# KristinnVikarJ/nbody-simulation

Measured on AMD Instinct MI355X. Metric: pair-interactions/sec + ms/step at N=1M direct O(N^2) (force + integration step), higher is better.
Workload: dtype f32; 1 GPU; direct O(N^2) f32, N=1048576 bodies, seeded 2-D Plummer sphere, masses 1, dt=0.1, clamp=0.001 (BASELINE.json configs[2]); n_bodies=1048576, targets_per_gpu=1048576, n_ranks=1, entry=one process per GPU (sharding.py over nbody_direct_{prep,run}_dev), exchange=none, arith=AUTO (FAST kernel; EXACT on hazardous positions)

## Files before the change

nbody-simulation_amd/csrc/direct_mutual.hip:

```cpp
#include <hip/hip_runtime.h>
#include <stdint.h>

#include "direct_kernels.h"
#include "mutual_schedule.h"

namespace nbody {

namespace {

typedef float v2f __attribute__((ext_vector_type(2)));

constexpr int kWaves = 8;

constexpr int kSlice = kMutualSlice;
constexpr int kSliceCouples = kSlice / 2;
constexpr int kChunks = kSliceCouples / 64;
constexpr float kMarker = 1e30f;

__device__ __forceinline__ bool gate_open(const DirectArgs& a) { return a.run_state < 0 || a.flags[kFlagState] == a.run_state; }

__device__ __forceinline__ float4 couple_or_marker(const float4* c, int64_t k, int64_t n_couples) {
  return k < n_couples ? c[k] : make_float4(kMarker, kMarker, kMarker, kMarker);
}

#define NB_PX(K, H, D) "v_pk_add_f32 v[" D "], v[184:185], %[tx" #K "] op_sel:[0," #H "] op_sel_hi:[1," #H "] neg_lo:[0,1] neg_hi:[0,1]\n\t"
#define NB_PY(K, H, D) "v_pk_add_f32 v[" D "], v[186:187], %[ty" #K "] op_sel:[0," #H "] op_sel_hi:[1," #H "] neg_lo:[0,1] neg_hi:[0,1]\n\t"
#define NB_SQ(DX, DY, Q) "v_pk_mul_f32 v[" Q "], v[" DX "], v[" DX "]\n\tv_pk_fma_f32 v[" Q "], v[" DY "], v[" DY "], v[" Q "]\n\t"
#define NB_AD(XL, XH, YL, YH, SL, SH) "v_add_f32_e64 v" SL ", |v" XL "|, |v" YL "|\n\tv_add_f32_e64 v" SH ", |v" XH "|, |v" YH "|\n\t"
#define NB_DN(S, Q) "v_pk_fma_f32 v[" S "], v[" S "], v[" Q "], %[b]\n\t"
#define NB_RC(SL, SH) "v_rcp_f32_e32 v" SL ", v" SL "\n\tv_rcp_f32_e32 v" SH ", v" SH "\n\t"
#define NB_AC(T, DX, DY, S)                                                                                                          \
  "v_pk_fma_f32 %[ax" #T "], v[" DX "], v[" S "], %[ax" #T "]\n\t"                                                                    \
  "v_pk_fma_f32 v[188:189], v[" DX "], v[" S "], v[188:189] neg_lo:[1,0,0] neg_hi:[1,0,0]\n\t"                                                  \
  "v_pk_fma_f32 %[ay" #T "], v[" DY "], v[" S "], %[ay" #T "]\n\t"                                                                    \
  "v_pk_fma_f32 v[190:191], v[" DY "], v[" S "], v[190:191] neg_lo:[1,0,0] neg_hi:[1,0,0]\n\t"
#define NB_HALF(K0, K1, K2, K3, T0, T1, T2, T3, T4, T5, T6, T7)                                                                    \
  NB_PX(K0, 0, "192:193") NB_PX(K0, 1, "200:201") NB_PX(K1, 0, "208:209") NB_PX(K1, 1, "216:217")                                   \
  NB_PX(K2, 0, "224:225") NB_PX(K2, 1, "232:233") NB_PX(K3, 0, "240:241") NB_PX(K3, 1, "248:249")                                   \
  NB_PY(K0, 0, "194:195") NB_PY(K0, 1, "202:203") NB_PY(K1, 0, "210:211") NB_PY(K1, 1, "218:219")                                   \
  NB_PY(K2, 0, "226:227") NB_PY(K2, 1, "234:235") NB_PY(K3, 0, "242:243") NB_PY(K3, 1, "250:251")                                   \
  NB_SQ("192:193", "194:195", "196:197") NB_SQ("200:201", "202:203", "204:205") NB_SQ("208:209", "210:211", "212:213")             \
  NB_SQ("216:217", "218:219", "220:221") NB_SQ("224:225", "226:227", "228:229") NB_SQ("232:233", "234:235", "236:237")             \
  NB_SQ("240:241", "242:243", "244:245") NB_SQ("248:249", "250:251", "252:253")                                                    \
  "s_setprio 0\n\t"                                                                                                                \
  NB_AD("192", "193", "194", "195", "198", "199") NB_AD("200", "201", "202", "203", "206", "207")                                  \
  NB_AD("208", "209", "210", "211", "214", "215") NB_AD("216", "217", "218", "219", "222", "223")                                  \
  NB_AD("224", "225", "226", "227", "230", "231") NB_AD("232", "233", "234", "235", "238", "239")                                  \
  NB_AD("240", "241", "242", "243", "246", "247") NB_AD("248", "249", "250", "251", "254", "255")                                  \
  "s_setprio 1\n\t"                                                                                                                \
  NB_DN("198:199", "196:197") NB_DN("206:207", "204:205") NB_DN("214:215", "212:213") NB_DN("222:223", "220:221")                 \
  NB_DN("230:231", "228:229") NB_DN("238:239", "236:237") NB_DN("246:247", "244:245") NB_DN("254:255", "252:253")                 \
  NB_RC("198", "199")                                                                                                              \
  NB_RC("206", "207") NB_AC(T0, "192:193", "194:195", "198:199")                                                                   \
  NB_RC("214", "215") NB_AC(T1, "200:201", "202:203", "206:207")                                                                   \
  NB_RC("222", "223") NB_AC(T2, "208:209", "210:211", "214:215")                                                                   \
  NB_RC("230", "231") NB_AC(T3, "216:217", "218:219", "222:223")                                                                   \
  NB_RC("238", "239") NB_AC(T4, "224:225", "226:227", "230:231")                                                                   \
  NB_RC("246", "247") NB_AC(T5, "232:233", "234:235", "238:239")                                                                   \
  NB_RC("254", "255") NB_AC(T6, "240:241", "242:243", "246:247")                                                                   \
  NB_AC(T7, "248:249", "250:251", "254:255")
#define NB_ROT(R) "v_mov_b32_dpp " R ", " R " wave_ror:1 row_mask:0xf bank_mask:0xf\n\t"

__device__ __forceinline__ void mutual_steps(const v2f* tx, const v2f* ty, v2f* ax, v2f* ay, float4& rc, float4& sacc, int steps,
                                             unsigned long long bias2) {
  asm volatile("v_mov_b32 v184, %[r0]\n\tv_mov_b32 v185, %[r1]\n\tv_mov_b32 v186, %[r2]\n\tv_mov_b32 v187, %[r3]\n\t"
               "v_mov_b32 v188, %[o0]\n\tv_mov_b32 v189, %[o1]\n\tv_mov_b32 v190, %[o2]\n\tv_mov_b32 v191, %[o3]\n\t"
               "s_mov_b32 s88, %[n]\n"
               ".Lnb_mutual_%=:\n\t"
               NB_HALF(0, 1, 2, 3, 0, 1, 2, 3, 4, 5, 6, 7) NB_HALF(4, 5, 6, 7, 8, 9, 10, 11, 12, 13, 14, 15)
               NB_ROT("v184") NB_ROT("v185") NB_ROT("v186") NB_ROT("v187") NB_ROT("v188") NB_ROT("v189") NB_ROT("v190") NB_ROT("v191")
               "s_sub_u32 s88, s88, 1\n\t"
               "s_cmp_lg_u32 s88, 0\n\t"
               "s_cbranch_scc1 .Lnb_mutual_%=\n\t"
               "v_mov_b32 %[o0], v188\n\tv_mov_b32 %[o1], v189\n\tv_mov_b32 %[o2], v190\n\tv_mov_b32 %[o3], v191\n\t"
               "v_mov_b32 %[r0], v184\n\tv_mov_b32 %[r1], v185\n\tv_mov_b32 %[r2], v186\n\tv_mov_b32 %[r3], v187\n\t"
               : [ax0] "+v"(ax[0]), [ax1] "+v"(ax[1]), [ax2] "+v"(ax[2]), [ax3] "+v"(ax[3]), [ax4] "+v"(ax[4]), [ax5] "+v"(ax[5]),
                 [ax6] "+v"(ax[6]), [ax7] "+v"(ax[7]), [ax8] "+v"(ax[8]), [ax9] "+v"(ax[9]), [ax10] "+v"(ax[10]), [ax11] "+v"(ax[11]),
                 [ax12] "+v"(ax[12]), [ax13] "+v"(ax[13]), [ax14] "+v"(ax[14]), [ax15] "+v"(ax[15]),
                 [ay0] "+v"(ay[0]), [ay1] "+v"(ay[1]), [ay2] "+v"(ay[2]), [ay3] "+v"(ay[3]), [ay4] "+v"(ay[4]), [ay5] "+v"(ay[5]),
                 [ay6] "+v"(ay[6]), [ay7] "+v"(ay[7]), [ay8] "+v"(ay[8]), [ay9] "+v"(ay[9]), [ay10] "+v"(ay[10]), [ay11] "+v"(ay[11]),
                 [ay12] "+v"(ay[12]), [ay13] "+v"(ay[13]), [ay14] "+v"(ay[14]), [ay15] "+v"(ay[15]),
                 [o0] "+v"(sacc.x), [o1] "+v"(sacc.y), [o2] "+v"(sacc.z), [o3] "+v"(sacc.w),
                 [r0] "+v"(rc.x), [r1] "+v"(rc.y), [r2] "+v"(rc.z), [r3] "+v"(rc.w)
               : [tx0] "v"(tx[0]), [tx1] "v"(tx[1]), [tx2] "v"(tx[2]), [tx3] "v"(tx[3]), [tx4] "v"(tx[4]), [tx5] "v"(tx[5]),
                 [tx6] "v"(tx[6]), [tx7] "v"(tx[7]), [ty0] "v"(ty[0]), [ty1] "v"(ty[1]), [ty2] "v"(ty[2]), [ty3] "v"(ty[3]),
                 [ty4] "v"(ty[4]), [ty5] "v"(ty[5]), [ty6] "v"(ty[6]), [ty7] "v"(ty[7]), [b] "s"(bias2), [n] "s"(steps)
               : "v184", "v185", "v186", "v187", "v188", "v189", "v190", "v191",
                 "v192", "v193", "v194", "v195", "v196", "v197", "v198", "v199", "v200", "v201", "v202", "v203", "v204", "v205",
                 "v206", "v207", "v208", "v209", "v210", "v211", "v212", "v213", "v214", "v215", "v216", "v217", "v218", "v219",
                 "v220", "v221", "v222", "v223", "v224", "v225", "v226", "v227", "v228", "v229", "v230", "v231", "v232", "v233",
                 "v234", "v235", "v236", "v237", "v238", "v239", "v240", "v241", "v242", "v243", "v244", "v245", "v246", "v247",
                 "v248", "v249", "v250", "v251", "v252", "v253", "v254", "v255", "s88", "scc");
}
#undef NB_PX
#undef NB_PY
#undef NB_SQ
#undef NB_AD
#undef NB_DN
#undef NB_RC
#undef NB_AC
#undef NB_HALF
#undef NB_ROT

__device__ __forceinline__ void load_targets(const float4* couples, int64_t n_couples, int s, int w, int lane, v2f* tx, v2f* ty) {
  const int64_t tc0 = (int64_t)s * kSliceCouples + 512 * w + 8 * lane;
#pragma unroll
  for (int k = 0; k < 8; ++k) {
    const float4 c = couple_or_marker(couples, tc0 + k, n_couples);
    tx[k] = v2f{c.x, c.y};
    ty[k] = v2f{c.z, c.w};
  }
}

__device__ __forceinline__ void zero_acc(v2f* ax, v2f* ay) {
#pragma unroll
  for (int t = 0; t < 16; ++t) ax[t] = ay[t] = v2f{0.f, 0.f};
}

__device__ __forceinline__ void add_chunk(const v2f* ax, const v2f* ay, float* tot_x, float* tot_y) {
#pragma unroll
  for (int t = 0; t < 16; ++t) {
    tot_x[t] += ax[t].x + ax[t].y;
    tot_y[t] += ay[t].x + ay[t].y;
  }
}

constexpr unsigned long long kBias2 = 0x1280000012800000ull;

__device__ __forceinline__ void off_item(const float4* couples, int64_t n_couples, int s, int b, int w, int lane, float4 (*red)[kWaves][64],
                                         float2* tpart, float2* spart_f2) {
  v2f tx[8], ty[8];
  load_targets(couples, n_couples, s, w, lane, tx, ty);
  float tot_x[16], tot_y[16];
#pragma unroll
  for (int t = 0; t < 16; ++t) tot_x[t] = tot_y[t] = 0.f;
  float* spart = reinterpret_cast<float*>(spart_f2);
  for (int c = 0; c < kChunks; ++c) {
    float4 rc = couple_or_marker(couples, (int64_t)b * kSliceCouples + 64 * c + lane, n_couples);
    v2f ax[16], ay[16];
    zero_acc(ax, ay);
    float4 sacc = make_float4(0.f, 0.f, 0.f, 0.f);
    mutual_steps(tx, ty, ax, ay, rc, sacc, 64, kBias2);
    add_chunk(ax, ay, tot_x, tot_y);
    red[c & 1][w][lane] = sacc;
    __syncthreads();
    if (threadIdx.x < 256) {
      const int q = threadIdx.x >> 2, comp = threadIdx.x & 3;
      float r = 0.f;
#pragma unroll
      for (int v = 0; v < kWaves; ++v) r += reinterpret_cast<const float*>(&red[c & 1][v][q])[comp];
      spart[(size_t)(128 * c + 2 * q + (comp & 1)) * 2 + (comp >> 1)] = r;
    }
  }
#pragma unroll
  for (int t = 0; t < 16; ++t) tpart[1024 * w + 16 * lane + t] = make_float2(tot_x[t], tot_y[t]);
}

__device__ __forceinline__ void diag_item(const float4* couples, int64_t n_couples, int s, int w, int lane, float4 (*src)[8][64],
                                          float2* out) {
  using namespace mutual_schedule;
  v2f tx[8], ty[8];
  load_targets(couples, n_couples, s, w, lane, tx, ty);
  float tot_x[16], tot_y[16];
#pragma unroll
  for (int t = 0; t < 16; ++t) tot_x[t] = tot_y[t] = 0.f;
  const int64_t c0 = (int64_t)s * kSliceCouples;
  for (int p = 0; p < kDiagPhases; ++p) {
    const int u = diag_block(w, p), r0 = diag_first_step(w, p), n = diag_steps(p);
    for (int j = 0; j < 8; ++j) {
      float4 rc = couple_or_marker(couples, c0 + 512 * u + 8 * ((lane - r0) & 63) + j, n_couples);
      v2f ax[16], ay[16];
      zero_acc(ax, ay);
      float4 sacc = make_float4(0.f, 0.f, 0.f, 0.f);
      int moved;
      if (p == 0) {
        mutual_steps(tx, ty, ax, ay, rc, sacc, 1, kBias2);
        sacc = make_float4(0.f, 0.f, 0.f, 0.f);
        mutual_steps(tx, ty, ax, ay, rc, sacc, n - 2, kBias2);
        const float4 keep = sacc;
        mutual_steps(tx, ty, ax, ay, rc, sacc, 1, kBias2);
        sacc = keep;
        moved = n - 1;
      } else {
        mutual_steps(tx, ty, ax, ay, rc, sacc, n, kBias2);
        moved = n;
      }
      add_chunk(ax, ay, tot_x, tot_y);
      const int shift = (r0 + moved) & 63;
      if (shift) {
        const int from = (lane + shift) & 63;
        sacc = make_float4(__shfl(sacc.x, from), __shfl(sacc.y, from), __shfl(sacc.z, from), __shfl(sacc.w, from));
      }
      float4& d = src[u][j][lane];
      if (p == 0) {
        d = sacc;
      } else {
        const float4 o = d;
        d = make_float4(o.x + sacc.x, o.y + sacc.y, o.z + sacc.z, o.w + sacc.w);
      }
    }
    __syncthreads();
  }
#pragma unroll
  for (int k = 0; k < 8; ++k) {
    const float4 q = src[w][k][lane];
    out[1024 * w + 16 * lane + 2 * k] = make_float2(tot_x[2 * k] + q.x, tot_y[2 * k] + q.z);
    out[1024 * w + 16 * lane + 2 * k + 1] = make_float2(tot_x[2 * k + 1] + q.y, tot_y[2 * k + 1] + q.w);
  }
  __syncthreads();
}

__global__ __launch_bounds__(kWaves * 64) void direct_mutual(const DirectArgs a, MutualArea m, int64_t lo) {
  if (!gate_open(a)) return;
  const int nb = m.n_slices;
  int s, b;
  mutual_schedule::unit_slices(lo + blockIdx.x, nb, s, b);
  const int lane = threadIdx.x & 63;
  const int w = __builtin_amdgcn_readfirstlane((int)(threadIdx.x >> 6));
  const float4* couples = reinterpret_cast<const float4*>(a.src_pos);
  const int64_t n_couples = a.n_src / 2;
  float2* tpart = m.tpart + (size_t)blockIdx.x * kSlice;
  float2* spart = m.spart + (size_t)blockIdx.x * kSlice;
  __shared__ float4 lds[8][8][64];
  __builtin_amdgcn_s_setprio(1);
  if (s < b) {
    off_item(couples, n_couples, s, b, w, lane, reinterpret_cast<float4(*)[kWaves][64]>(&lds[0][0][0]), tpart, spart);
  } else {
    diag_item(couples, n_couples, s, w, lane, lds, tpart);
    if (s + 1 < nb) diag_item(couples, n_couples, s + 1, w, lane, lds, spart);
  }
}

__global__ __launch_bounds__(256) void direct_mutual_near(const DirectArgs a, MutualArea m) {
  if (!gate_open(a)) return;
  const int n_near = a.flags[kFlagNearCount];
  const float4* couples = reinterpret_cast<const float4*>(a.src_pos);
  const int n_couples = a.n_src / 2;
  const int per = (n_couples + kMutualNearSplit - 1) / kMutualNearSplit;
  const int q0 = blockIdx.x * per, q1 = q0 + per < n_couples ? q0 + per : n_couples;
  __shared__ float2 red[256];
  for (int k = blockIdx.y; k < n_near; k += gridDim.y) {
    const float2 p = a.pos_all[a.near_list[k]];
    float ax = 0.f, ay = 0.f;
#pragma unroll 4
    for (int q = q0 + (int)threadIdx.x; q < q1; q += 256) {
      const float4 c = couples[q];
#pragma unroll
      for (int h = 0; h < 2; ++h) {
        const float dx = (h ? c.y : c.x) - p.x, dy = (h ? c.w : c.z) - p.y;
        const float sum = __builtin_fabsf(dx) + __builtin_fabsf(dy);
        const float d2 = __builtin_fmaf(dy, dy, dx * dx);
        const float s = __builtin_amdgcn_rcpf(__builtin_fmaf(sum, d2, 8.0779356694631609e-28f));
        ax = __builtin_fmaf(dx, s, ax);
        ay = __builtin_fmaf(dy, s, ay);
      }
    }
    red[threadIdx.x] = make_float2(ax, ay);
    __syncthreads();
    for (int w = 128; w > 0; w >>= 1) {
      if ((int)threadIdx.x < w) {
        red[threadIdx.x].x += red[threadIdx.x + w].x;
        red[threadIdx.x].y += red[threadIdx.x + w].y;
      }
      __syncthreads();
    }
    if (threadIdx.x == 0) m.near_part[(size_t)k * kMutualNearSplit + blockIdx.x] = red[0];
    __syncthreads();
  }
}

__global__ __launch_bounds__(256) void direct_mutual_reduce(const DirectArgs a, MutualArea m, int64_t lo, int64_t hi, int first, int last) {
  using mutual_schedule::item_of;
  if (!gate_open(a)) return;
  const int i = blockIdx.x * 256 + threadIdx.x;
  if (i >= a.n_tgt) return;
  const int nb = m.n_slices;
  const int s = i / kSlice, l = i % kSlice;
  int r0 = 0, r1 = s;
  while (r0 < r1) {
    const int mid = (r0 + r1) >> 1;
    if (item_of(mid, s, nb) < lo) r0 = mid + 1; else r1 = mid;
  }
  int re = s;
  r1 = r0;
  while (r1 < re) {
    const int mid = (r1 + re) >> 1;
    if (item_of(mid, s, nb) < hi) r1 = mid + 1; else re = mid;
  }
  const int64_t b0 = s + 1 < nb ? item_of(s, s + 1, nb) : 0, b1 = s + 1 < nb ? item_of(s, nb - 1, nb) + 1 : 0;
  const int64_t w0 = b0 > lo ? b0 : lo, w1 = b1 < hi ? b1 : hi;
  const int64_t d = mutual_schedule::diag_unit(s, nb);
  const bool has_d = d >= lo && d < hi;
  if (r0 == r1 && w0 >= w1 && !has_d && !first && !last) return;
  float2 acc = first ? make_float2(0.f, 0.f) : a.partial[i];
#pragma unroll 8
  for (int r = r0; r < r1; ++r) {
    const float2 p = m.spart[(size_t)(item_of(r, s, nb) - lo) * kSlice + l];
    acc.x += p.x;
    acc.y += p.y;
  }
#pragma unroll 8
  for (int64_t it = w0; it < w1; ++it) {
    const float2 p = m.tpart[(size_t)(it - lo) * kSlice + l];
    acc.x += p.x;
    acc.y += p.y;
  }
  if (has_d) {
    const float2 p = ((s & 1) ? m.spart : m.tpart)[(size_t)(d - lo) * kSlice + l];
    acc.x += p.x;
    acc.y += p.y;
  }
  if (last) {
    if (m.is_near[i]) {
      const float2* np = m.near_part + (size_t)m.near_scan[i] * kMutualNearSplit;
      acc = np[0];
      for (int g = 1; g < kMutualNearSplit; ++g) {
        acc.x += np[g].x;
        acc.y += np[g].y;
      }
    }
    acc = make_float2(acc.x * a.uniform_mass, acc.y * a.uniform_mass);
  }
  a.partial[i] = acc;
}

}

int mutual_slices(int64_t n_slots) { return (int)((n_slots + kSlice - 1) / kSlice); }

size_t mutual_area_bytes(int64_t n_src) {
  return 2 * (size_t)kMutualStripItems * kSlice * sizeof(float2) + ((size_t)n_src / 64 + 2) * kMutualNearSplit * sizeof(float2);
}

MutualArea mutual_area(void* base, int64_t n_src, const uint32_t* is_near, const uint32_t* near_scan) {
  MutualArea m{};
  m.n_slices = mutual_slices(far_padded(n_src));
  float2* p = (float2*)base;
  m.tpart = p;
  p += (size_t)kMutualStripItems * kSlice;
  m.spart = p;
  p += (size_t)kMutualStripItems * kSlice;
  m.near_part = p;
  m.is_near = is_near;
  m.near_scan = near_scan;
  return m;
}

hipError_t launch_direct_mutual(hipStream_t s, const DirectArgs& a, const MutualArea& m) {
  if (a.n_tgt <= 0) return hipSuccess;
  if (!a.src_couples || a.tgt_begin != 0 || a.n_src < a.n_tgt || m.n_slices != mutual_slices(a.n_src)) return hipErrorInvalidValue;
  int dev = 0, cus = 0;
  hipError_t e = hipGetDevice(&dev);
  if (e == hipSuccess) e = hipDeviceGetAttribute(&cus, hipDeviceAttributeMultiprocessorCount, dev);
  if (e != hipSuccess) return e;
  if (cus <= 0) return hipErrorInvalidValue;
  const int64_t units = mutual_schedule::units(m.n_slices);
  const int64_t strip = mutual_schedule::strip_units(cus, kMutualStripItems);
  const dim3 rgrid((unsigned)((a.n_tgt + 255) / 256));
  hipLaunchKernelGGL(direct_mutual_near, dim3(kMutualNearSplit, kMutualNearRows), dim3(256), 0, s, a, m);
  for (int64_t lo = 0; lo < units; lo += strip) {
    const int64_t hi = lo + strip < units ? lo + strip : units;
    hipLaunchKernelGGL(direct_mutual, dim3((unsigned)(hi - lo)), dim3(kWaves * 64), 0, s, a, m, lo);
    hipLaunchKernelGGL(direct_mutual_reduce, rgrid, dim3(256), 0, s, a, m, lo, hi, lo == 0 ? 1 : 0, hi == units ? 1 : 0);
  }
  return hipGetLastError();
}

}
```

Measured before the change: 9989 billion pair-interactions/s.

## Rotate mutual ring via ds_bpermute overlapped with compute and prefetch next couple

The per-step ring rotation of source couples and their reaction accumulators moves from DPP wave_ror moves, placed after the compute, to ds_bpermute issued in the middle of the step and waited on later, so the LDS-crossbar permutes can overlap with the FMA/RCP work. The inline asm now binds operands directly to fixed registers instead of copying them in and out. The next chunk's couple is loaded one iteration ahead to hide global-load latency. The change adds LDS permute traffic and waitcnt stalls, and narrows indices to 32-bit with a new n_src guard.

```diff
diff --git a/nbody-simulation_amd/csrc/direct_mutual.hip b/nbody-simulation_amd/csrc/direct_mutual.hip
--- a/nbody-simulation_amd/csrc/direct_mutual.hip
+++ b/nbody-simulation_amd/csrc/direct_mutual.hip
@@ -21,6 +21,16 @@
 
 __device__ __forceinline__ float4 couple_or_marker(const float4* c, int64_t k, int64_t n_couples) {
   return k < n_couples ? c[k] : make_float4(kMarker, kMarker, kMarker, kMarker);
+}
+
+struct Ahead {
+  float4 v;
+  bool past;
+  __device__ __forceinline__ float4 couple() const { return past ? make_float4(kMarker, kMarker, kMarker, kMarker) : v; }
+};
+__device__ __forceinline__ Ahead couple_ahead(const float4* c, int k, int n_couples) {
+  const bool past = k >= n_couples;
+  return Ahead{c[past ? 0 : k], past};
 }
 
 #define NB_PX(K, H, D) "v_pk_add_f32 v[" D "], v[184:185], %[tx" #K "] op_sel:[0," #H "] op_sel_hi:[1," #H "] neg_lo:[0,1] neg_hi:[0,1]\n\t"
@@ -34,11 +44,11 @@
   "v_pk_fma_f32 v[188:189], v[" DX "], v[" S "], v[188:189] neg_lo:[1,0,0] neg_hi:[1,0,0]\n\t"                                                  \
   "v_pk_fma_f32 %[ay" #T "], v[" DY "], v[" S "], %[ay" #T "]\n\t"                                                                    \
   "v_pk_fma_f32 v[190:191], v[" DY "], v[" S "], v[190:191] neg_lo:[1,0,0] neg_hi:[1,0,0]\n\t"
-#define NB_HALF(K0, K1, K2, K3, T0, T1, T2, T3, T4, T5, T6, T7)                                                                    \
+#define NB_HALF(K0, K1, K2, K3, T0, T1, T2, T3, T4, T5, T6, T7, MID, PRE)                                                                  \
   NB_PX(K0, 0, "192:193") NB_PX(K0, 1, "200:201") NB_PX(K1, 0, "208:209") NB_PX(K1, 1, "216:217")                                   \
   NB_PX(K2, 0, "224:225") NB_PX(K2, 1, "232:233") NB_PX(K3, 0, "240:241") NB_PX(K3, 1, "248:249")                                   \
   NB_PY(K0, 0, "194:195") NB_PY(K0, 1, "202:203") NB_PY(K1, 0, "210:211") NB_PY(K1, 1, "218:219")                                   \
-  NB_PY(K2, 0, "226:227") NB_PY(K2, 1, "234:235") NB_PY(K3, 0, "242:243") NB_PY(K3, 1, "250:251")                                   \
+  NB_PY(K2, 0, "226:227") NB_PY(K2, 1, "234:235") NB_PY(K3, 0, "242:243") NB_PY(K3, 1, "250:251") MID                               \
   NB_SQ("192:193", "194:195", "196:197") NB_SQ("200:201", "202:203", "204:205") NB_SQ("208:209", "210:211", "212:213")             \
   NB_SQ("216:217", "218:219", "220:221") NB_SQ("224:225", "226:227", "228:229") NB_SQ("232:233", "234:235", "236:237")             \
   NB_SQ("240:241", "242:243", "244:245") NB_SQ("248:249", "250:251", "252:253")                                                    \
@@ -51,7 +61,7 @@
   NB_DN("198:199", "196:197") NB_DN("206:207", "204:205") NB_DN("214:215", "212:213") NB_DN("222:223", "220:221")                 \
   NB_DN("230:231", "228:229") NB_DN("238:239", "236:237") NB_DN("246:247", "244:245") NB_DN("254:255", "252:253")                 \
   NB_RC("198", "199")                                                                                                              \
-  NB_RC("206", "207") NB_AC(T0, "192:193", "194:195", "198:199")                                                                   \
+  NB_RC("206", "207") PRE NB_AC(T0, "192:193", "194:195", "198:199")                                                                   \
   NB_RC("214", "215") NB_AC(T1, "200:201", "202:203", "206:207")                                                                   \
   NB_RC("222", "223") NB_AC(T2, "208:209", "210:211", "214:215")                                                                   \
   NB_RC("230", "231") NB_AC(T3, "216:217", "218:219", "222:223")                                                                   \
@@ -60,33 +70,49 @@
   NB_RC("254", "255") NB_AC(T6, "240:241", "242:243", "246:247")                                                                   \
   NB_AC(T7, "248:249", "250:251", "254:255")
 #define NB_ROT(R) "v_mov_b32_dpp " R ", " R " wave_ror:1 row_mask:0xf bank_mask:0xf\n\t"
-
-__device__ __forceinline__ void mutual_steps(const v2f* tx, const v2f* ty, v2f* ax, v2f* ay, float4& rc, float4& sacc, int steps,
-                                             unsigned long long bias2) {
-  asm volatile("v_mov_b32 v184, %[r0]\n\tv_mov_b32 v185, %[r1]\n\tv_mov_b32 v186, %[r2]\n\tv_mov_b32 v187, %[r3]\n\t"
-               "v_mov_b32 v188, %[o0]\n\tv_mov_b32 v189, %[o1]\n\tv_mov_b32 v190, %[o2]\n\tv_mov_b32 v191, %[o3]\n\t"
-               "s_mov_b32 s88, %[n]\n"
+#define NB_PRM(R) "ds_bpermute_b32 " R ", %[from], " R "\n\t"
+#ifndef NBODY_MUTUAL_RING
+#define NBODY_MUTUAL_RING 2
+#endif
+#if NBODY_MUTUAL_RING == 0
+#define NB_TOP ""
+#define NB_PRE ""
+#define NB_MID ""
+#define NB_END NB_ROT("v184") NB_ROT("v185") NB_ROT("v186") NB_ROT("v187") NB_ROT("v188") NB_ROT("v189") NB_ROT("v190") NB_ROT("v191")
+#elif NBODY_MUTUAL_RING == 1
+#define NB_TOP "s_waitcnt lgkmcnt(0)\n\t"
+#define NB_PRE ""
+#define NB_MID NB_PRM("v184") NB_PRM("v185") NB_PRM("v186") NB_PRM("v187")
+#define NB_END NB_ROT("v188") NB_ROT("v189") NB_ROT("v190") NB_ROT("v191")
+#else
+#define NB_TOP "s_waitcnt lgkmcnt(4)\n\t"
+#define NB_PRE "s_waitcnt lgkmcnt(0)\n\t"
+#define NB_MID NB_PRM("v184") NB_PRM("v185") NB_PRM("v186") NB_PRM("v187")
+#define NB_END NB_PRM("v188") NB_PRM("v189") NB_PRM("v190") NB_PRM("v191")
+#endif
+
+__device__ __forceinline__ void mutual_steps(const v2f* tx, const v2f* ty, v2f* ax, v2f* ay, v2f& rx, v2f& ry, v2f& sax, v2f& say,
+                                             int steps, int from, unsigned long long bias2) {
+  asm volatile("s_mov_b32 s88, %[n]\n\t"
+               "s_waitcnt lgkmcnt(0)\n"
                ".Lnb_mutual_%=:\n\t"
-               NB_HALF(0, 1, 2, 3, 0, 1, 2, 3, 4, 5, 6, 7) NB_HALF(4, 5, 6, 7, 8, 9, 10, 11, 12, 13, 14, 15)
-               NB_ROT("v184") NB_ROT("v185") NB_ROT("v186") NB_ROT("v187") NB_ROT("v188") NB_ROT("v189") NB_ROT("v190") NB_ROT("v191")
+               NB_TOP NB_HALF(0, 1, 2, 3, 0, 1, 2, 3, 4, 5, 6, 7, "", NB_PRE) NB_HALF(4, 5, 6, 7, 8, 9, 10, 11, 12, 13, 14, 15, NB_MID, "")
+               NB_END
                "s_sub_u32 s88, s88, 1\n\t"
                "s_cmp_lg_u32 s88, 0\n\t"
                "s_cbranch_scc1 .Lnb_mutual_%=\n\t"
-               "v_mov_b32 %[o0], v188\n\tv_mov_b32 %[o1], v189\n\tv_mov_b32 %[o2], v190\n\tv_mov_b32 %[o3], v191\n\t"
-               "v_mov_b32 %[r0], v184\n\tv_mov_b32 %[r1], v185\n\tv_mov_b32 %[r2], v186\n\tv_mov_b32 %[r3], v187\n\t"
+               "s_waitcnt lgkmcnt(0)\n\t"
                : [ax0] "+v"(ax[0]), [ax1] "+v"(ax[1]), [ax2] "+v"(ax[2]), [ax3] "+v"(ax[3]), [ax4] "+v"(ax[4]), [ax5] "+v"(ax[5]),
                  [ax6] "+v"(ax[6]), [ax7] "+v"(ax[7]), [ax8] "+v"(ax[8]), [ax9] "+v"(ax[9]), [ax10] "+v"(ax[10]), [ax11] "+v"(ax[11]),
                  [ax12] "+v"(ax[12]), [ax13] "+v"(ax[13]), [ax14] "+v"(ax[14]), [ax15] "+v"(ax[15]),
                  [ay0] "+v"(ay[0]), [ay1] "+v"(ay[1]), [ay2] "+v"(ay[2]), [ay3] "+v"(ay[3]), [ay4] "+v"(ay[4]), [ay5] "+v"(ay[5]),
                  [ay6] "+v"(ay[6]), [ay7] "+v"(ay[7]), [ay8] "+v"(ay[8]), [ay9] "+v"(ay[9]), [ay10] "+v"(ay[10]), [ay11] "+v"(ay[11]),
                  [ay12] "+v"(ay[12]), [ay13] "+v"(ay[13]), [ay14] "+v"(ay[14]), [ay15] "+v"(ay[15]),
-                 [o0] "+v"(sacc.x), [o1] "+v"(sacc.y), [o2] "+v"(sacc.z), [o3] "+v"(sacc.w),
-                 [r0] "+v"(rc.x), [r1] "+v"(rc.y), [r2] "+v"(rc.z), [r3] "+v"(rc.w)
+                 "+{v[184:185]}"(rx), "+{v[186:187]}"(ry), "+{v[188:189]}"(sax), "+{v[190:191]}"(say)
                : [tx0] "v"(tx[0]), [tx1] "v"(tx[1]), [tx2] "v"(tx[2]), [tx3] "v"(tx[3]), [tx4] "v"(tx[4]), [tx5] "v"(tx[5]),
                  [tx6] "v"(tx[6]), [tx7] "v"(tx[7]), [ty0] "v"(ty[0]), [ty1] "v"(ty[1]), [ty2] "v"(ty[2]), [ty3] "v"(ty[3]),
-                 [ty4] "v"(ty[4]), [ty5] "v"(ty[5]), [ty6] "v"(ty[6]), [ty7] "v"(ty[7]), [b] "s"(bias2), [n] "s"(steps)
-               : "v184", "v185", "v186", "v187", "v188", "v189", "v190", "v191",
-                 "v192", "v193", "v194", "v195", "v196", "v197", "v198", "v199", "v200", "v201", "v202", "v203", "v204", "v205",
+                 [ty4] "v"(ty[4]), [ty5] "v"(ty[5]), [ty6] "v"(ty[6]), [ty7] "v"(ty[7]), [b] "s"(bias2), [n] "s"(steps), [from] "v"(from)
+               : "v192", "v193", "v194", "v195", "v196", "v197", "v198", "v199", "v200", "v201", "v202", "v203", "v204", "v205",
                  "v206", "v207", "v208", "v209", "v210", "v211", "v212", "v213", "v214", "v215", "v216", "v217", "v218", "v219",
                  "v220", "v221", "v222", "v223", "v224", "v225", "v226", "v227", "v228", "v229", "v230", "v231", "v232", "v233",
                  "v234", "v235", "v236", "v237", "v238", "v239", "v240", "v241", "v242", "v243", "v244", "v245", "v246", "v247",
@@ -101,6 +127,11 @@
 #undef NB_AC
 #undef NB_HALF
 #undef NB_ROT
+#undef NB_PRM
+#undef NB_TOP
+#undef NB_PRE
+#undef NB_MID
+#undef NB_END
 
 __device__ __forceinline__ void load_targets(const float4* couples, int64_t n_couples, int s, int w, int lane, v2f* tx, v2f* ty) {
   const int64_t tc0 = (int64_t)s * kSliceCouples + 512 * w + 8 * lane;
@@ -135,14 +166,19 @@
 #pragma unroll
   for (int t = 0; t < 16; ++t) tot_x[t] = tot_y[t] = 0.f;
   float* spart = reinterpret_cast<float*>(spart_f2);
+  const int from = 4 * ((lane - 1) & 63);
+  const int b0 = b * kSliceCouples + lane, nc = (int)n_couples;
+  Ahead nxt = couple_ahead(couples, b0, nc);
   for (int c = 0; c < kChunks; ++c) {
-    float4 rc = couple_or_marker(couples, (int64_t)b * kSliceCouples + 64 * c + lane, n_couples);
+    const float4 rc = nxt.couple();
+    v2f rx = v2f{rc.x, rc.y}, ry = v2f{rc.z, rc.w};
+    if (c + 1 < kChunks) nxt = couple_ahead(couples, b0 + 64 * (c + 1), nc);
     v2f ax[16], ay[16];
     zero_acc(ax, ay);
-    float4 sacc = make_float4(0.f, 0.f, 0.f, 0.f);
-    mutual_steps(tx, ty, ax, ay, rc, sacc, 64, kBias2);
+    v2f sax = v2f{0.f, 0.f}, say = v2f{0.f, 0.f};
+    mutual_steps(tx, ty, ax, ay, rx, ry, sax, say, 64, from, kBias2);
     add_chunk(ax, ay, tot_x, tot_y);
-    red[c & 1][w][lane] = sacc;
+    red[c & 1][w][lane] = make_float4(sax.x, sax.y, say.x, say.y);
     __syncthreads();
     if (threadIdx.x < 256) {
       const int q = threadIdx.x >> 2, comp = threadIdx.x & 3;
@@ -164,28 +200,38 @@
   float tot_x[16], tot_y[16];
 #pragma unroll
   for (int t = 0; t < 16; ++t) tot_x[t] = tot_y[t] = 0.f;
-  const int64_t c0 = (int64_t)s * kSliceCouples;
+  const int c0 = s * kSliceCouples, nc = (int)n_couples;
+  const int from1 = 4 * ((lane - 1) & 63);
+  auto chunk_couple = [&](int q) {
+    const int p = q >> 3, j = q & 7;
+    return c0 + 512 * diag_block(w, p) + 8 * ((lane - diag_first_step(w, p)) & 63) + j;
+  };
+  Ahead nxt = couple_ahead(couples, chunk_couple(0), nc);
   for (int p = 0; p < kDiagPhases; ++p) {
     const int u = diag_block(w, p), r0 = diag_first_step(w, p), n = diag_steps(p);
     for (int j = 0; j < 8; ++j) {
-      float4 rc = couple_or_marker(couples, c0 + 512 * u + 8 * ((lane - r0) & 63) + j, n_couples);
+      const float4 rc = nxt.couple();
+      v2f rx = v2f{rc.x, rc.y}, ry = v2f{rc.z, rc.w};
+      if (8 * p + j + 1 < 8 * kDiagPhases) nxt = couple_ahead(couples, chunk_couple(8 * p + j + 1), nc);
       v2f ax[16], ay[16];
       zero_acc(ax, ay);
-      float4 sacc = make_float4(0.f, 0.f, 0.f, 0.f);
+      v2f sax = v2f{0.f, 0.f}, say = v2f{0.f, 0.f};
       int moved;
       if (p == 0) {
-        mutual_steps(tx, ty, ax, ay, rc, sacc, 1, kBias2);
-        sacc = make_float4(0.f, 0.f, 0.f, 0.f);
-        mutual_steps(tx, ty, ax, ay, rc, sacc, n - 2, kBias2);
-        const float4 keep = sacc;
-        mutual_steps(tx, ty, ax, ay, rc, sacc, 1, kBias2);
-        sacc = keep;
+        mutual_steps(tx, ty, ax, ay, rx, ry, sax, say, 1, from1, kBias2);
+        sax = say = v2f{0.f, 0.f};
+        mutual_steps(tx, ty, ax, ay, rx, ry, sax, say, n - 2, from1, kBias2);
+        const v2f keep_x = sax, keep_y = say;
+        mutual_steps(tx, ty, ax, ay, rx, ry, sax, say, 1, from1, kBias2);
+        sax = keep_x;
+        say = keep_y;
         moved = n - 1;
       } else {
-        mutual_steps(tx, ty, ax, ay, rc, sacc, n, kBias2);
+        mutual_steps(tx, ty, ax, ay, rx, ry, sax, say, n, from1, kBias2);
         moved = n;
       }
       add_chunk(ax, ay, tot_x, tot_y);
+      float4 sacc = make_float4(sax.x, sax.y, say.x, say.y);
       const int shift = (r0 + moved) & 63;
       if (shift) {
         const int from = (lane + shift) & 63;
@@ -348,7 +394,7 @@
 
 hipError_t launch_direct_mutual(hipStream_t s, const DirectArgs& a, const MutualArea& m) {
   if (a.n_tgt <= 0) return hipSuccess;
-  if (!a.src_couples || a.tgt_begin != 0 || a.n_src < a.n_tgt || m.n_slices != mutual_slices(a.n_src)) return hipErrorInvalidValue;
+  if (!a.src_couples || a.tgt_begin != 0 || a.n_src < a.n_tgt || a.n_src < 2 || a.n_src > INT32_MAX || m.n_slices != mutual_slices(a.n_src)) return hipErrorInvalidValue;
   int dev = 0, cus = 0;
   hipError_t e = hipGetDevice(&dev);
   if (e == hipSuccess) e = hipDeviceGetAttribute(&cus, hipDeviceAttributeMultiprocessorCount, dev);
```

Result: slower. 9667 billion pair-interactions/s (-3.2%).
